# rohitsinghlab/SAME

Hardware: AMD Instinct MI355X
Metric: cell-pairs/sec on 100k×100k cost build + edge-cross sweep; % HBM roofline (higher is better)
Workload: dtype f64

## Files before the change

include/same_hip.h:

```cpp
#ifndef SAME_HIP_H
#define SAME_HIP_H

#include <stddef.h>
#include <stdint.h>

#ifdef __cplusplus
extern "C" {
#endif

#define SAME_OK 0
#define SAME_EINVAL (-22)
#define SAME_ENOMEM (-12)
#define SAME_EIO (-5)
#define SAME_ENODEV (-19)
#define SAME_ERANGE (-34)
#define SAME_EUNSURE (-11)

#define SAME_ABI_VERSION 8
#define SAME_MAX_KNN 448
#define SAME_MAX_TYPES 4096

typedef struct same_ctx same_ctx;
typedef struct same_sweep same_sweep;

// ... 128 lines not shown
                       int64_t Tr, const int32_t *dmatch, double *dout_before, double *dout_after,
                       uint8_t *dout_matched3, uint8_t *dout_flipped);
int same_xyorder_sweep_dev(same_ctx *ctx, const double *daxy, int64_t n_m, const double *drxy,
                           const int32_t *dtris, int64_t Tr, const int32_t *dmatch,
                           uint8_t *dedge_flags, uint8_t *dtri_flag, uint8_t *dpoint_flag,
                           uint64_t *dcounts);
int same_orient_sweep_dev(same_sweep *sweep, const int32_t *dmatch, int64_t *out_checked,
                          int32_t *out_viol_idx, int64_t *out_nviol);
int same_orient_flags_dev(same_sweep *sweep, const int32_t *dmatch, int64_t t_begin, int64_t t_end,
                          uint8_t *dflag);
int same_orient_from_flags_dev(same_sweep *sweep, const uint8_t *dflag, int64_t *out_checked,
                               int32_t *out_viol_idx, int64_t *out_nviol);
int same_first_candidate_dev(same_ctx *ctx, const int32_t *didx, int64_t rows, int k, int32_t *dmatch);

#define SAME_WINDOW_BATCH_MAX 64
typedef struct same_section same_section;
typedef struct same_window same_window;
enum {
    SAME_WINDOW_ALIGNED_XY = 0,
    SAME_WINDOW_ALIGNED_ROWS = 1,
    SAME_WINDOW_ROWS_M = 2,
    SAME_WINDOW_ROWS_R = 3,
    SAME_WINDOW_PAIRS = 4,
    SAME_WINDOW_COSTS = 5,
    SAME_WINDOW_KEPT = 6,
    SAME_WINDOW_SIGNS = 7,
    SAME_WINDOW_WEIGHTS = 8,
    SAME_WINDOW_MATCH = 9,
    SAME_WINDOW_TRIANGLES = 10
};
// ... 94 lines not shown
```

include/same_hip_diag.h:

```cpp
#ifndef SAME_HIP_DIAG_H
#define SAME_HIP_DIAG_H

#include "same_hip.h"

#ifdef __cplusplus
extern "C" {
#endif

enum { SAME_STAT_LAUNCHES = 0, SAME_STAT_FILLS = 1, SAME_STAT_COPIES = 2, SAME_STAT_WAITS = 3, SAME_STAT_GREEDY_READBACKS = 4, SAME_STAT_COUNT = 5 };
int same_ctx_stat(same_ctx *ctx, int which, int64_t *out);


int same_timer_start(same_ctx *ctx);
int same_timer_stop(same_ctx *ctx, float *out_ms);
int same_timer_mark(same_ctx *ctx);
int same_timer_read(same_ctx *ctx, float *out_ms);

int same_ctx_pci_bus_id(same_ctx *ctx, char *out, size_t out_len);
int same_dev_mem_info(same_ctx *ctx, int64_t *out_free, int64_t *out_total);

#define SAME_SPREAD_INFO_LEN 14
int same_dev_alloc_spread(same_ctx *ctx, size_t bytes, void **out_dptr, int64_t *out_info);

#define SAME_Q32_MAX_TYPES 32
int same_quantize_u32_dev(same_ctx *ctx, const double *dsrc, int64_t n, double offset, double scale,
// ... 13 lines not shown
```

same_amd/_lib.py:

```python
import ctypes
import os
import sys
import threading

import numpy as np

_HERE = os.path.dirname(os.path.abspath(__file__))
LIB_PATH = os.environ.get("SAME_HIP_LIB") or os.path.join(_HERE, "libsame_hip.so")

c_i64 = ctypes.c_int64
c_int = ctypes.c_int
c_dbl = ctypes.c_double
c_flt = ctypes.c_float
c_vp = ctypes.c_void_p
c_sz = ctypes.c_size_t

UNIQUE_ID_BYTES = 128
ABI_VERSION = 8
DT_U8, DT_I32, DT_U64, DT_F64 = 0, 1, 2, 3
OP_SUM, OP_MAX, OP_MIN = 0, 1, 2
SPREAD_INFO_LEN = 14
MAX_KNN = 448
MAX_TYPES = 4096

_PROTOTYPES = {
    "same_abi_version": [],
    "same_device_count": [ctypes.POINTER(c_int)],
    "same_ctx_create": [c_int, ctypes.POINTER(c_vp)],
    "same_ctx_destroy": [c_vp],
    "same_ctx_sync": [c_vp],
    "same_strerror": [c_int],
    "same_last_error": [c_vp],
    "same_ctx_info": [c_vp, ctypes.c_char_p, c_sz, ctypes.POINTER(c_int), ctypes.POINTER(c_i64)],
    "same_ctx_pci_bus_id": [c_vp, ctypes.c_char_p, c_sz],
    "same_ctx_stat": [c_vp, c_int, ctypes.POINTER(c_i64)],
    "same_dev_alloc": [c_vp, c_sz, ctypes.POINTER(c_vp)],
    "same_dev_free": [c_vp, c_vp],
    "same_dev_alloc_spread": [c_vp, c_sz, ctypes.POINTER(c_vp), ctypes.POINTER(c_i64)],
    "same_h2d": [c_vp, c_vp, c_vp, c_sz],
    "same_d2h": [c_vp, c_vp, c_vp, c_sz],
    "same_dev_memset": [c_vp, c_vp, c_int, c_sz],
    "same_d2d": [c_vp, c_vp, c_vp, c_sz],
    "same_dev_mem_info": [c_vp, ctypes.POINTER(c_i64), ctypes.POINTER(c_i64)],
    "same_ctx_release_scratch": [c_vp],
    "same_timer_start": [c_vp],
    "same_timer_stop": [c_vp, ctypes.POINTER(c_flt)],
    "same_timer_mark": [c_vp],
    "same_timer_read": [c_vp, ctypes.POINTER(c_flt)],
    "same_pair_cost_f64": [c_vp, c_vp, c_vp, c_i64, c_i64, c_int, c_vp, c_vp, c_vp, c_i64, c_dbl, c_vp],
    "same_pair_cost_f32": [c_vp, c_vp, c_vp, c_i64, c_i64, c_int, c_vp, c_vp, c_vp, c_i64, c_flt, c_vp],
# ... 73 lines not shown
    "same_comm_destroy": [c_vp],
    "same_allgather_dev": [c_vp, c_vp, c_vp, c_sz],
    "same_allgather_dev_async": [c_vp, c_vp, c_vp, c_sz],
    "same_comm_wait": [c_vp],
    "same_allreduce_dev": [c_vp, c_vp, c_sz, c_int, c_int],
    "same_comm_group_start": [c_vp],
    "same_comm_group_end": [c_vp],
    "same_comm_info": [c_vp, ctypes.POINTER(c_int), ctypes.POINTER(c_int), ctypes.POINTER(c_int)],
    "same_comm_device": [c_vp, ctypes.POINTER(c_int)],
    "same_comm_gather_time": [c_vp, ctypes.POINTER(c_flt), ctypes.POINTER(c_i64)],
}
EXPORTS = tuple(_PROTOTYPES)


SAME_EINVAL, SAME_ENOMEM, SAME_EIO, SAME_ENODEV, SAME_ERANGE, SAME_EUNSURE = -22, -12, -5, -19, -34, -11
SAME_DD_FEW_POINTS, SAME_DD_NO_ANGLE, SAME_DD_NONFINITE, SAME_DD_IN_DOUBT, SAME_DD_OVERFLOW = 1, 2, 4, 8, 16


class SameHipError(RuntimeError):

    def __init__(self, code, what, detail=""):
        self.code = code
        super().__init__(f"{what}: {detail}" if detail else what)


_lib = None
_lib_lock = threading.Lock()


def load():
# ... 213 lines not shown
```

same_amd/csrc/common.h:

```cpp
#pragma once
#include <hip/hip_runtime.h>

#include <cstdint>
#include <cstdio>
#include <cstring>
#include <string>
#include <vector>

#include "same_hip_diag.h"

struct ncclComm;

enum Slot {
    SL_A = 0, SL_R, SL_AXY, SL_RXY, SL_PAIRS, SL_OUT0, SL_OUT1, SL_OUT2, SL_TRIS, SL_MATCH,
    SL_SIGN, SL_SIZE, SL_TYPE, SL_FLAG0, SL_FLAG1, SL_FLAG2, SL_COUNTS, SL_X, SL_MASK,
    SL_K_HIST, SL_K_RANK, SL_K_SXY, SL_K_SIDX, SL_K_BBOX, SL_K_START,
    SL_COUNT
};

struct same_spread_alloc {
    char *va = nullptr;
    size_t bytes = 0;
    std::vector<void *> handles;
};
void same_spread_release(same_spread_alloc &a);

struct same_ctx {
    int device = -1;
    hipStream_t stream = nullptr;
    hipStream_t comm_stream = nullptr;
    hipEvent_t ev0 = nullptr, ev1 = nullptr;
    hipEvent_t ev_ready = nullptr, ev_gathered = nullptr;
    hipEvent_t ev_gather0 = nullptr;
    bool gather_open = false, gather_stamped = false, in_group = false;
    size_t gather_bytes = 0;
    void *slot[SL_COUNT] = {};
    size_t slot_bytes[SL_COUNT] = {};
    void *pinned = nullptr;
    size_t pinned_bytes = 0;
    std::string err;
    int cu_count = 0;
    ncclComm *comm = nullptr;
    int nranks = 1, rank = 0;
    std::vector<same_spread_alloc> spread;
    int64_t stats[SAME_STAT_COUNT] = {};
};

#define SAME_LAUNCH(ctx, kernel, grid, block, lds, ...)                                  \
    do {                                                                                 \
        ++(ctx)->stats[SAME_STAT_LAUNCHES];                                              \
        hipLaunchKernelGGL(kernel, grid, block, lds, (ctx)->stream, __VA_ARGS__);        \
    } while (0)
#define SAME_FILL(ctx, ptr, value, bytes)                                                \
    do {                                                                                 \
// ... 67 lines not shown
    void *p = nullptr;
    int rc = same_slot(ctx, s, n * sizeof(T), &p);
    *out = static_cast<T *>(p);
    return rc;
}
template <typename T>
inline int up_as(same_ctx *ctx, Slot s, const T *host, size_t n, T **out) {
    void *p = nullptr;
    int rc = same_up(ctx, s, host, n * sizeof(T), &p);
    *out = static_cast<T *>(p);
    return rc;
}

static inline int64_t ceil_div(int64_t a, int64_t b) { return (a + b - 1) / b; }

int check_index_range(same_ctx *ctx, const int32_t *idx, int64_t n, int64_t lo, int64_t hi, const char *what);

int same_pair_rowmin_core(same_ctx *ctx, const int32_t *dpairs, const double *dcosts, int64_t P, int64_t n_m, double *dout);
int same_greedy_core(same_ctx *ctx, const int32_t *dpairs, const double *dcosts, int64_t P, int64_t n_m, int64_t n_r,
                     const uint8_t *dprefer, int32_t *dmatch_pair, int *out_rounds);

constexpr int SAME_GREEDY_BATCH_MAX = 64;
struct same_greedy_state {
    uint8_t *alive = nullptr;
    uint8_t *used = nullptr;
    unsigned long long *key[2] = {nullptr, nullptr};
    unsigned *idx[2] = {nullptr, nullptr};
    unsigned long long *sel = nullptr;
    bool float_costs = false;
};
// ... 38 lines not shown
```

same_amd/csrc/ctx.hip:

```cpp
#include "common.h"

extern "C" {

int same_abi_version(void) { return SAME_ABI_VERSION; }

int same_device_count(int *out_count) {
    if (!out_count) return SAME_EINVAL;
    int n = 0;
    hipError_t e = hipGetDeviceCount(&n);
    if (e != hipSuccess) { *out_count = 0; return SAME_ENODEV; }
    *out_count = n;
    return SAME_OK;
}

int same_ctx_create(int device, same_ctx **out) {
    if (!out) return SAME_EINVAL;
    *out = nullptr;
    int n = 0;
    if (hipGetDeviceCount(&n) != hipSuccess || n <= 0) return SAME_ENODEV;
    if (device < 0 || device >= n) return SAME_EINVAL;
    same_ctx *ctx = new (std::nothrow) same_ctx();
    if (!ctx) return SAME_ENOMEM;
    ctx->device = device;
    hipError_t e = hipSetDevice(device);
// ... 13 lines not shown
    ctx->cu_count = prop.multiProcessorCount;
    *out = ctx;
    return SAME_OK;
}

void same_ctx_destroy(same_ctx *ctx) {
    if (!ctx) return;
    (void)hipSetDevice(ctx->device);
    if (ctx->comm) same_comm_destroy(ctx);
    if (ctx->stream) (void)hipStreamSynchronize(ctx->stream);
    if (ctx->comm_stream) (void)hipStreamSynchronize(ctx->comm_stream);
    for (int s = 0; s < SL_COUNT; ++s)
        if (ctx->slot[s]) (void)hipFree(ctx->slot[s]);
    for (auto &a : ctx->spread) same_spread_release(a);
    if (ctx->pinned) (void)hipHostFree(ctx->pinned);
    if (ctx->ev0) (void)hipEventDestroy(ctx->ev0);
    if (ctx->ev1) (void)hipEventDestroy(ctx->ev1);
    if (ctx->ev_ready) (void)hipEventDestroy(ctx->ev_ready);
    if (ctx->ev_gathered) (void)hipEventDestroy(ctx->ev_gathered);
    if (ctx->ev_gather0) (void)hipEventDestroy(ctx->ev_gather0);
    if (ctx->comm_stream) (void)hipStreamDestroy(ctx->comm_stream);
    if (ctx->stream) (void)hipStreamDestroy(ctx->stream);
    delete ctx;
}

int same_ctx_sync(same_ctx *ctx) {
    REQUIRE(ctx, ctx != nullptr);
    SAME_TRY(same_use(ctx));
    HIP_TRY(ctx, hipStreamSynchronize(ctx->stream));
    HIP_TRY(ctx, hipStreamSynchronize(ctx->comm_stream));
// ... 25 lines not shown
    return SAME_OK;
}

int same_ctx_pci_bus_id(same_ctx *ctx, char *out, size_t out_len) {
    REQUIRE(ctx, ctx && out && out_len >= 16 && out_len <= 4096);
    HIP_TRY(ctx, hipDeviceGetPCIBusId(out, (int)out_len, ctx->device));
    return SAME_OK;
}

int same_ctx_stat(same_ctx *ctx, int which, int64_t *out) {
    REQUIRE(ctx, ctx && out && which >= 0 && which < SAME_STAT_COUNT);
    *out = ctx->stats[which];
    return SAME_OK;
}

int same_dev_alloc(same_ctx *ctx, size_t bytes, void **out_dptr) {
    REQUIRE(ctx, ctx && out_dptr);
    SAME_TRY(same_use(ctx));
    *out_dptr = nullptr;
    HIP_TRY(ctx, hipMalloc(out_dptr, bytes ? bytes : 1));
    return SAME_OK;
}

int same_dev_free(same_ctx *ctx, void *dptr) {
    REQUIRE(ctx, ctx != nullptr);
    SAME_TRY(same_use(ctx));
    HIP_TRY(ctx, hipStreamSynchronize(ctx->stream));
    for (size_t i = 0; i < ctx->spread.size(); ++i)
        if (ctx->spread[i].va == dptr) {
            same_spread_release(ctx->spread[i]);
// ... 136 lines not shown
```

same_amd/csrc/window_finish.hip:

```cpp
#include "assign.h"
#include "refine.h"

namespace {

using namespace devmath;
using namespace win;
using scan::Pair;

struct FilterArgs {
    const double *xy;
    const int32_t *raw;
    int64_t Tr, n;
    const int32_t *type_id;
    uint8_t *cls;
    double *perim;
    uint8_t *has_kept, *any_valid;
    unsigned long long *best_p;
    unsigned *best_t, *first_v;
    unsigned long long *st_keep, *st_own, *counters;
    int32_t *klist, *nlist, *out;
};

__global__ __launch_bounds__(256) void filter_classify_kernel(Batch<FilterArgs> b, double radius, int angle_enabled, double cos_thr, int near_enabled,
                                                               double tol) {
    const FilterArgs &w = b.w[blockIdx.y];
    if ((int64_t)blockIdx.x * blockDim.x >= w.Tr) return;
    const int64_t t = (int64_t)blockIdx.x * blockDim.x + threadIdx.x;
    const int32_t *__restrict__ tris = w.raw, *__restrict__ type_id = w.type_id;
    bool near = false;
    if (t < w.Tr) {
        const int32_t a = tris[3 * t], bb = tris[3 * t + 1], d = tris[3 * t + 2];
        const TriClass r = classify_triangle(ld2(w.xy, a), ld2(w.xy, bb), ld2(w.xy, d), radius, angle_enabled, cos_thr,
                                             type_id && type_id[a] == type_id[bb] && type_id[bb] == type_id[d]);
        w.cls[t] = r.cls;
        w.perim[t] = r.perim;
        near = near_enabled && r.cls != 1 && fabs(r.maxcos - cos_thr) <= tol;
        if (r.cls == 0 || r.cls == 3) {
            w.any_valid[a] = 1; w.any_valid[bb] = 1; w.any_valid[d] = 1;
            if (r.cls == 0) { w.has_kept[a] = 1; w.has_kept[bb] = 1; w.has_kept[d] = 1; }
        }
        if (w.best_p && r.cls == 3) {
            const unsigned long long key = ~(unsigned long long)__double_as_longlong(r.perim);
            atomicMax(&w.best_p[a], key); atomicMax(&w.best_p[bb], key); atomicMax(&w.best_p[d], key);
        }
    }
    const unsigned long long nb = __ballot(near);
    if ((threadIdx.x & 63) == 0 && nb) atomicAdd(&w.counters[FC_NEAR], (unsigned long long)__builtin_popcountll(nb));
}
__global__ __launch_bounds__(scan::NT) void filter_keep_kernel(Batch<FilterArgs> b) {
    __shared__ scan::Shared sh;
    const FilterArgs &w = b.w[blockIdx.y];
    const int nb = (int)scan::blocks_for(w.Tr);
    if ((int)blockIdx.x >= nb || w.Tr == 0) return;
    const int64_t Tr = w.Tr;
    const uint8_t *__restrict__ cls = w.cls;
    auto val = [&](int64_t t) { return Pair{t < Tr && cls[t] == 0 ? 1u : 0u, 0u}; };
    Pair through;
    const Pair off = scan::exclusive(w.st_keep, (int)blockIdx.x, val, sh, &through);
    const int64_t t = (int64_t)blockIdx.x * scan::NT + threadIdx.x;
    if (t < Tr) {
        const uint8_t c = cls[t];
        if (c == 0) w.klist[off.a] = (int32_t)t;
// ... 182 lines not shown
    __syncthreads();
    if (threadIdx.x < 7) {
        const int s = part[0][threadIdx.x] + part[1][threadIdx.x] + part[2][threadIdx.x] + part[3][threadIdx.x];
        if (s) atomicAdd(&counters[threadIdx.x < 6 ? threadIdx.x : SC_TIES], (unsigned long long)s);
    }
}

struct FilterPlan {
    FilterArgs args{};
    void *zero = nullptr;
    size_t zero_bytes = 0;
    unsigned long long *counters = nullptr;
    bool readd = false;
};

int prepare_filter(same_window *w, const int32_t *d_simplices, int64_t Tr, int ignore_same_type, int ensure_min_triangle_per_node, FilterPlan *plan) {
    same_ctx *ctx = w->ctx;
    const int64_t n = w->n_ua;
    const bool use_type = ignore_same_type && w->has_type;
    plan->readd = use_type && ensure_min_triangle_per_node;
    Carver cv;
    const size_t st_keep = scan::status_bytes(Tr), st_own = scan::status_bytes(n);
    const size_t o_st_keep = cv.take(st_keep), o_st_own = cv.take(st_own), o_counters = cv.take(64), o_has_kept = cv.take((size_t)n),
                 o_any_valid = cv.take((size_t)n), o_best_p = cv.take((size_t)n * 8), o_best_t = cv.take((size_t)n * 4),
                 o_first_v = cv.take((size_t)Tr * 4);
    const size_t zero_bytes = cv.off;
    const size_t o_cls = cv.take((size_t)Tr), o_perim = cv.take((size_t)Tr * 8), o_klist = cv.take((size_t)Tr * 4), o_nlist = cv.take((size_t)n * 4);
    SAME_TRY(ensure(ctx, w->filter, cv.off));
    SAME_TRY(ensure(ctx, w->tris, (size_t)std::max<int64_t>(Tr, 1) * 12));
    char *base = static_cast<char *>(w->filter.p);
    auto at = [&](size_t off) { return base + off; };
    unsigned long long *dc = reinterpret_cast<unsigned long long *>(at(o_counters));
    plan->counters = dc;
    FilterArgs &a = plan->args;
    a.xy = w->axy_c;
    a.raw = d_simplices;
    a.Tr = Tr;
    a.n = n;
    a.type_id = use_type ? w->type_c : nullptr;
    a.cls = reinterpret_cast<uint8_t *>(at(o_cls));
    a.perim = reinterpret_cast<double *>(at(o_perim));
    a.has_kept = reinterpret_cast<uint8_t *>(at(o_has_kept));
    a.any_valid = reinterpret_cast<uint8_t *>(at(o_any_valid));
    a.best_p = plan->readd ? reinterpret_cast<unsigned long long *>(at(o_best_p)) : nullptr;
    a.best_t = reinterpret_cast<unsigned *>(at(o_best_t));
    a.first_v = reinterpret_cast<unsigned *>(at(o_first_v));
    a.st_keep = scan::arg(reinterpret_cast<unsigned long long *>(at(o_st_keep)));
    a.st_own = scan::arg(reinterpret_cast<unsigned long long *>(at(o_st_own)));
    a.counters = dc;
    a.klist = reinterpret_cast<int32_t *>(at(o_klist));
// ... 275 lines not shown
                if (q < batch) break;
                if (batch < SAME_GREEDY_BATCH_MAX) batch *= 2;
            }
            again = true;
        }
    }
    SAME_TRY(settle(w, p, again));
    for (int q = 0; q < 8; ++q) out_stats[q] = (int64_t)cnt[q];
    out_stats[SC_ROUNDS] = rounds;
    *out_ties += (int64_t)cnt[SC_TIES];
    memcpy(out_match_row, h + p->o_match_row, (size_t)n * sizeof(int32_t));
    memcpy(out_point_flag, h + p->o_pflag, (size_t)n);
    return SAME_OK;
}

int filter_finish(same_window *const *windows, int n_windows, const int32_t *simplices, const int64_t *simplex_offsets, int prefiltered,
                  bool on_device, double radius, int angle_enabled, double cos_thr, double near_tol, int ignore_same_type,
                  int ensure_min_triangle_per_node, double no_match_penalty, int32_t *out_match_row, uint8_t *out_point_flag,
                  int64_t *out_stats, int64_t *out_counts) {
    same_ctx *ctx = nullptr;
    SAME_TRY(check_batch(windows, n_windows, &ctx));
    REQUIRE(ctx, simplex_offsets && out_counts && out_stats && simplex_offsets[0] == 0);
    int64_t n_cells = 0;
    for (int i = 0; i < n_windows; ++i) {
        const int64_t Tr = simplex_offsets[i + 1] - simplex_offsets[i];
        REQUIRE(ctx, windows[i]->staged == 2 && Tr >= 0 && Tr < ((int64_t)1 << 31) - 512);
        n_cells += windows[i]->n_ua;
    }
    REQUIRE(ctx, (simplex_offsets[n_windows] == 0 || simplices || on_device) && (n_cells == 0 || (out_match_row && out_point_flag)));
    for (int q = 0; q < 4 * n_windows; ++q) out_counts[q] = 0;
    for (int q = 0; q < 8 * n_windows; ++q) out_stats[q] = 0;
    SAME_TRY(same_use(ctx));
    if (!on_device)
        for (int i = 0; i < n_windows; ++i)
            SAME_TRY(check_index_range(ctx, simplices + 3 * simplex_offsets[i], (simplex_offsets[i + 1] - simplex_offsets[i]) * 3, 0,
                                       windows[i]->n_ua, "triangles"));
    struct Item {
        FilterPlan fplan;
        FinishPlan plan;
        bool filtered = false, enqueued = false;
    };
    std::vector<Item> items((size_t)n_windows);
    const int32_t *d_simplices = nullptr;
    if (!on_device && !prefiltered && simplex_offsets[n_windows] > 0) {
        int32_t *d = nullptr;
        SAME_TRY(slot_as(ctx, SL_TRIS, (size_t)simplex_offsets[n_windows] * 3, &d));
        SAME_COPY(ctx, d, simplices, (size_t)simplex_offsets[n_windows] * 12, hipMemcpyHostToDevice);
        d_simplices = d;
    }
    int rc = SAME_OK;
    std::vector<same_window *> live;
    std::vector<FinishPlan *> plans;
    std::vector<FilterPlan *> fplans;
    for (int i = 0; i < n_windows && rc == SAME_OK; ++i) {
        same_window *w = windows[i];
        Item &it = items[(size_t)i];
        const int32_t *tri = on_device ? nullptr : simplices + 3 * simplex_offsets[i];
        const int64_t Tr = simplex_offsets[i + 1] - simplex_offsets[i];
        w->filtered = w->finished = 0;
        w->Tr = 0;
        w->as_rounds = w->as_flags = 0;
        w->as_objective = 0.0;
        w->rf_rounds = w->rf_moves = w->rf_settled = 0;
        w->rf_obj0 = w->rf_obj = 0.0;
        w->rf_nm = no_match_penalty;
        if (w->n_ua == 0) continue;
        if (Tr && !prefiltered) {
            const int32_t *raw = on_device ? static_cast<const int32_t *>(w->dd_tris.p) : d_simplices + 3 * simplex_offsets[i];
            rc = prepare_filter(w, raw, Tr, ignore_same_type, ensure_min_triangle_per_node, &it.fplan);
            if (rc == SAME_OK) rc = prepare_finish(w, nullptr, Tr, it.fplan.counters + FC_TR, &it.plan);
            if (rc == SAME_OK) {
                fplans.push_back(&it.fplan);
                it.plan.filter_zero = it.fplan.zero;
                it.plan.filter_zero_bytes = it.fplan.zero_bytes;
            }
            it.filtered = true;
        } else {
            rc = prepare_finish(w, Tr ? tri : nullptr, Tr, nullptr, &it.plan);
        }
        if (rc == SAME_OK) {
            live.push_back(w);
            plans.push_back(&it.plan);
        }
    }
    for (size_t g = 0; g < live.size() && rc == SAME_OK; g += SAME_LAUNCH_WINDOWS) {
        ZeroArgs zr[SAME_LAUNCH_WINDOWS];
        const int n_g = (int)std::min<size_t>(SAME_LAUNCH_WINDOWS, live.size() - g);
        for (int q = 0; q < n_g; ++q) {
            const FinishPlan *fp = plans[g + (size_t)q];
            zr[q] = ZeroArgs{{fp->zero, fp->filter_zero}, {fp->zero_bytes, fp->filter_zero_bytes}};
        }
        rc = launch_zero(ctx, zr, n_g);
    }
    for (size_t g = 0, e; g < fplans.size() && rc == SAME_OK; g = e) {
        for (e = g + 1; e < fplans.size() && e - g < SAME_LAUNCH_WINDOWS && fplans[e]->readd == fplans[g]->readd; ++e) {}
        rc = launch_filter(ctx, fplans.data() + g, (int)(e - g), radius, angle_enabled, cos_thr, near_tol);
    }
    for (size_t g = 0, e; g < live.size() && rc == SAME_OK; g = e) {
        for (e = g + 1; e < live.size() && e - g < SAME_LAUNCH_WINDOWS && live[e]->cost_f32 == live[g]->cost_f32 &&
// ... 20 lines not shown
                    }
                    if (rc == SAME_OK) rc = enqueue_finish_copy(w, &it.plan);
                }
                it.enqueued = rc == SAME_OK;
            }
            if (rc == SAME_OK && n_g && (n_g == SAME_LAUNCH_WINDOWS || i == n_windows - 1)) {
                rc = launch_copy_back(ctx, ca, n_g);
                n_g = 0;
            }
        }
    }
    if (rc != SAME_OK) {
        (void)hipStreamSynchronize(ctx->stream);
        return rc;
    }
    SAME_WAIT(ctx);
    int64_t cell0 = 0;
    for (int i = 0; i < n_windows; ++i) {
        same_window *w = windows[i];
        Item &it = items[(size_t)i];
        const int64_t Tr = simplex_offsets[i + 1] - simplex_offsets[i];
        int64_t *counts = out_counts + 4 * i, *stats = out_stats + 8 * i;
        if (!it.enqueued) {
            w->filtered = w->finished = 1;
            continue;
        }
        int32_t *const match_out = out_match_row + cell0;
        uint8_t *const flag_out = out_point_flag + cell0;
        cell0 += w->n_ua;
        if (it.filtered) {
            const unsigned long long *hf = reinterpret_cast<const unsigned long long *>(static_cast<const char *>(w->host) + w->host_filter_off);
// ... 2 lines not shown
            counts[1] = n_add;
            counts[2] = n_near;
            counts[3] = (int64_t)hf[FC_TIES];
            if (n_near) {
                for (int q = 0; q < 8; ++q) stats[q] = 0;
                continue;
            }
            w->Tr = n_keep + n_add;
        } else {
            counts[0] = Tr;
            w->Tr = Tr;
        }
        SAME_TRY(read_finish(w, &it.plan, match_out, flag_out, stats, counts + 3));
        w->filtered = w->finished = 1;
    }
    return SAME_OK;
}

}

extern "C" {

int same_window_filter_finish(same_window *const *windows, int n_windows, const int32_t *simplices, const int64_t *simplex_offsets, int prefiltered,
                              double radius, int angle_enabled, double cos_thr, double near_tol, int ignore_same_type,
                              int ensure_min_triangle_per_node, double no_match_penalty, int32_t *out_match_row, uint8_t *out_point_flag,
                              int64_t *out_stats, int64_t *out_counts) {
    return filter_finish(windows, n_windows, simplices, simplex_offsets, prefiltered, false, radius, angle_enabled, cos_thr, near_tol,
                         ignore_same_type, ensure_min_triangle_per_node, no_match_penalty, out_match_row, out_point_flag, out_stats, out_counts);
}

int same_window_filter_finish_device(same_window *const *windows, int n_windows, double radius, int angle_enabled, double cos_thr, double near_tol,
                                     int ignore_same_type, int ensure_min_triangle_per_node, double no_match_penalty, int32_t *out_match_row,
                                     uint8_t *out_point_flag, int64_t *out_stats, int64_t *out_counts) {
    same_ctx *ctx = nullptr;
    SAME_TRY(check_batch(windows, n_windows, &ctx));
    std::vector<int64_t> offsets((size_t)n_windows + 1, 0);
    for (int i = 0; i < n_windows; ++i) {
        REQUIRE(ctx, windows[i]->dd_ok && windows[i]->staged == 2);
        offsets[(size_t)i + 1] = offsets[(size_t)i] + windows[i]->n_dd;
    }
    return filter_finish(windows, n_windows, nullptr, offsets.data(), 0, true, radius, angle_enabled, cos_thr, near_tol, ignore_same_type,
                         ensure_min_triangle_per_node, no_match_penalty, out_match_row, out_point_flag, out_stats, out_counts);
}
// ... 66 lines not shown
```

same_amd/csrc/window_internal.h:

```cpp
#pragma once
#include <algorithm>
#include <cmath>
#include <memory>
#include <mutex>
#include <new>
#include <shared_mutex>
#include <utility>
#include <vector>

#include "common.h"
#include "devmath.h"
#include "scan.h"

struct same_knn_index;
extern "C" int same_knn_index_build(same_ctx *ctx, const double *drxy, int64_t n_r, double radius, same_knn_index **out);
extern "C" void same_knn_index_destroy(same_knn_index *ix);

namespace win {

constexpr int MAX_RUN_CELLS = 64;
constexpr int64_t MAX_GRID_CELLS = (int64_t)1 << 22;
constexpr unsigned OUTSIDE = 0x80000000u;

struct DevBuf {
// ... 41 lines not shown
struct Batch {
    A w[SAME_LAUNCH_WINDOWS];
};

struct ZeroArgs {
    void *p[2];
    size_t bytes[2];
};

struct CopyArgs {
    const void *src[2];
    void *dst[2];
    size_t bytes[2];
};

struct Cover {
    int cx0 = 0, ncx = 0, cy0 = 0, ncy = 0;
    int64_t n_cand = 0;
    bool aligned = false, use_runs = false;
};

enum { FC_KEEP = 0, FC_ADD = 1, FC_NEAR = 2, FC_TR = 3, FC_TIES = 4, FC_COPIED = 5 };
enum { SC_CHECKED = 0, SC_FLIPPED = 1, SC_CMP = 2, SC_VIOL = 3, SC_TVIOL = 4, SC_AFLIP = 5, SC_ROUNDS = 6, SC_MATCHED = 7, SC_REMAINING = 8, SC_TIES = 9,
       SC_REFINE = 16, SC_COUNT = 32 };

}

struct same_section {
    same_ctx *ctx = nullptr;
    int64_t n = 0;
    int T = 0;
    int cost_f32 = 0;
    double *xy = nullptr;
    void *xy_c = nullptr;
    void *types_c = nullptr;
    double *types64 = nullptr;
    double *size = nullptr;
// ... 57 lines not shown
```

same_amd/csrc/window_stage.hip:

```cpp
#include "window_internal.h"

namespace {

using namespace devmath;
using namespace win;
using scan::Pair;

__global__ __launch_bounds__(256) void zero_kernel(Batch<ZeroArgs> b) {
    const ZeroArgs &w = b.w[blockIdx.y];
    typedef unsigned u4 __attribute__((ext_vector_type(4)));
#pragma unroll
    for (int r = 0; r < 2; ++r) {
        const size_t n16 = w.bytes[r] >> 4;
        u4 *dst = static_cast<u4 *>(w.p[r]);
        for (size_t i = (size_t)blockIdx.x * blockDim.x + threadIdx.x; i < n16; i += (size_t)gridDim.x * blockDim.x) dst[i] = u4{0u, 0u, 0u, 0u};
        if (blockIdx.x == 0 && threadIdx.x < (w.bytes[r] & 15)) static_cast<char *>(w.p[r])[(n16 << 4) + threadIdx.x] = 0;
    }
}

__global__ __launch_bounds__(256) void copy_back_kernel(Batch<CopyArgs> b) {
    const CopyArgs &w = b.w[blockIdx.y];
    typedef unsigned u4 __attribute__((ext_vector_type(4)));
#pragma unroll
    for (int r = 0; r < 2; ++r) {
// ... 535 lines not shown
    REQUIRE(ctx, w->n_m <= w->cap_m && w->n_r <= w->cap_r && w->n_ua <= w->n_m && w->P <= (int64_t)sp.slots);
    out_counts[0] = w->n_m;
    out_counts[1] = w->n_r;
    out_counts[2] = w->n_ua;
    out_counts[3] = w->P;
    w->staged = (w->n_m && w->n_r) ? 2 : 1;
    return SAME_OK;
}

}

extern "C" {

int same_window_stage(same_window *const *windows, int n_windows, const same_section *mov, const same_section *ref, const double *boxes,
                      double radius, int k, double dist_ct_coeff, int64_t *out_counts) {
    same_ctx *ctx = nullptr;
    SAME_TRY(check_batch(windows, n_windows, &ctx));
    REQUIRE(ctx, mov && ref && boxes && out_counts && mov->ctx->device == ctx->device && ref->ctx->device == ctx->device);
    REQUIRE(ctx, mov->T == ref->T && mov->cost_f32 == ref->cost_f32 && k >= 1 && k <= SAME_MAX_KNN && radius >= 0.0);
    SAME_TRY(same_use(ctx));
    for (int i = 0; i < 4 * n_windows; ++i) out_counts[i] = 0;
    for (int i = 0; i < n_windows; ++i) windows[i]->staged = windows[i]->finished = windows[i]->filtered = windows[i]->dd_ok = 0;
    std::shared_ptr<same_knn_index> ix;
    SAME_TRY(knn_index_for(ctx, ref, radius, &ix));
    std::shared_lock<std::shared_mutex> grid_m(const_cast<same_section *>(mov)->grid_lock), grid_r;
    if (ref != mov) grid_r = std::shared_lock<std::shared_mutex>(const_cast<same_section *>(ref)->grid_lock);
    std::vector<StagePlan> plans((size_t)n_windows);
    int rc = SAME_OK;
    for (int i = 0; i < n_windows && rc == SAME_OK; ++i) rc = prepare_stage(windows[i], mov, ref, boxes + 4 * i, k, &plans[(size_t)i]);
    for (int g = 0; g < n_windows && rc == SAME_OK; g += SAME_LAUNCH_WINDOWS) {
// ... 11 lines not shown
            if (w->host_dev) {
                ca[q] = CopyArgs{{w->counts, nullptr}, {w->host_dev, nullptr}, {plans[(size_t)(g + q)].back_bytes, 0}};
                continue;
            }
            hipError_t e = hipMemcpyAsync(w->host, w->counts, plans[(size_t)(g + q)].back_bytes, hipMemcpyDeviceToHost, ctx->stream);
            ++ctx->stats[SAME_STAT_COPIES];
            if (e != hipSuccess) rc = same_fail(ctx, SAME_EIO, "stage copy back", e);
        }
        if (rc == SAME_OK) rc = launch_copy_back(ctx, ca, n_g);
    }
    if (rc != SAME_OK) {
        (void)hipStreamSynchronize(ctx->stream);
        for (int i = 0; i < n_windows; ++i) windows[i]->staged = 0;
        return rc;
    }
    SAME_WAIT(ctx);
    for (int i = 0; i < n_windows; ++i) SAME_TRY(collect_stage(windows[i], plans[(size_t)i], out_counts + 4 * i));
    return SAME_OK;
}

int same_window_fetch(same_window *w, int what, void *out, int64_t bytes) {
    if (!w) return SAME_EINVAL;
    same_ctx *ctx = w->ctx;
    REQUIRE(ctx, w->staged >= 1 && bytes >= 0 && (bytes == 0 || out));
    SAME_TRY(same_use(ctx));
    const char *h = static_cast<const char *>(w->host);
    const void *dev = nullptr;
    const void *host = nullptr;
    int64_t want = 0;
    const int64_t n_m = w->n_m, n_r = w->n_r, n_ua = w->n_ua, P = w->P, Tr = w->Tr;
    const bool full = w->staged == 2;
// ... 27 lines not shown
```

same_amd/delaunay.py:

```python
import os
import threading
from concurrent.futures import ThreadPoolExecutor

import numpy as np

from . import _lib, qhull_pool

GUARD = 16.0


def mode(optim_params=None):
    m = (optim_params or {}).get("hip_delaunay") or os.environ.get("SAME_DELAUNAY") or "qhull"
    m = str(m).lower()
    if m not in ("native", "device", "qhull"):
        raise ValueError(f"hip_delaunay / SAME_DELAUNAY must be 'native', 'device' or 'qhull', not {m!r}")
    return m


def device_filtered_triangles(points, radius, min_angle_deg, ctx=None, guard=GUARD, with_status=False):
    import ctypes

    from . import ops
    from .triangles import cos_threshold

    ctx = ops._ctx(ctx)
    pts = np.ascontiguousarray(points, dtype=np.float64).reshape(-1, 2)
    n = len(pts)
    angle_enabled, cos_thr = cos_threshold(min_angle_deg)
    out = np.empty((max(2 * n, 1), 3), np.int32)
    n_tris, status = ctypes.c_int64(0), ctypes.c_int(0)
    with ctx.lock:
        ctx.check(ctx.lib.same_delaunay_filtered(ctx.handle, pts.ctypes.data, n, float(abs(radius)), int(angle_enabled), float(cos_thr),
                                                 float(guard), out.ctypes.data, len(out), ctypes.byref(n_tris), ctypes.byref(status)),
                  "same_delaunay_filtered")
    tris = None if status.value else out[:n_tris.value].copy()
    return (tris, status.value) if with_status else tris


def native_simplices(points, guard=GUARD, with_margin=False):
    import ctypes

    lib = _lib.load()
    pts = np.ascontiguousarray(points, dtype=np.float64).reshape(-1, 2)
    n = len(pts)
    out = np.empty((max(2 * n - 5, 1), 3), np.int32)
    n_tris, margin = ctypes.c_int64(0), ctypes.c_double(0.0)
    rc = lib.same_delaunay2d(pts.ctypes.data, n, out.ctypes.data, len(out), ctypes.byref(n_tris), float(guard), ctypes.byref(margin))
    if rc == _lib.SAME_EUNSURE:
        return (None, margin.value) if with_margin else None
    if rc != 0:
        raise _lib.SameHipError(rc, "same_delaunay2d")
    tris = out[:n_tris.value]
    return (tris, margin.value) if with_margin else tris


class Ticket:

    def __init__(self, owner, points, pending=None, simplices=None, native=False, key=None):
        self.owner, self.points, self.key = owner, points, key
        self._pending, self._simplices, self.native = pending, simplices, native
# ... 172 lines not shown
```

same_amd/windows.py:

```python
import os

import numpy as np

from . import ops
from .delaunay import QHULL, QhullTriangulator, Ticket


def window_grid(ref_xy, mov_xy, window_size, overlap):
    import warnings

    with warnings.catch_warnings():
        warnings.simplefilter("ignore", RuntimeWarning)
        x_min = min(np.nanmin(ref_xy[:, 0]), np.nanmin(mov_xy[:, 0]))
        x_max = max(np.nanmax(ref_xy[:, 0]), np.nanmax(mov_xy[:, 0]))
        y_min = min(np.nanmin(ref_xy[:, 1]), np.nanmin(mov_xy[:, 1]))
        y_max = max(np.nanmax(ref_xy[:, 1]), np.nanmax(mov_xy[:, 1]))
    step = window_size - overlap
    xs = list(range(int(x_min), int(x_max), step))
    ys = list(range(int(y_min), int(y_max), step))
    return xs, ys, (x_min, x_max, y_min, y_max)


def _candidate_boxes(xs, ys, ws):
    boxes = np.empty((len(xs), len(ys), 4, 4), np.float64)
# ... 625 lines not shown

def stage_windows(states, moving, ref, boxes, radius, knn, dist_ct_coeff):
    ctx, n = states[0].ctx, len(states)
    boxes = np.ascontiguousarray(boxes, dtype=np.float64).reshape(n, 4)
    counts = np.zeros((n, 4), np.int64)
    with ctx.lock:
        ctx.check(ctx.lib.same_window_stage(_handles(states), n, moving.handle, ref.handle, boxes.ctypes.data, float(radius), int(knn),
                                            float(dist_ct_coeff), counts.ctypes.data), "same_window_stage")
    for s, c in zip(states, counts.tolist()):
        s.counts, s.n_triangles = tuple(c), 0
    return [s.counts for s in states]


def filter_finish_windows(states, simplices, radius, angle_enabled, cos_thr, near_tol, ignore_same_type, no_match_penalty,
                          ensure_min_triangle_per_node=True, prefiltered=False):
    ctx, n = states[0].ctx, len(states)
    tris = [ops._tris(t) for t in simplices]
    offsets = np.zeros(n + 1, np.int64)
    np.cumsum([len(t) for t in tris], out=offsets[1:])
    flat = tris[0] if n == 1 else np.concatenate(tris)

    def call(match_row, flag, stats, counts):
        return ctx.lib.same_window_filter_finish(_handles(states), n, flat.ctypes.data, offsets.ctypes.data, int(bool(prefiltered)),
                                                 float(radius),
                                                 int(angle_enabled), float(cos_thr), float(near_tol), int(bool(ignore_same_type)),
                                                 int(bool(ensure_min_triangle_per_node)), float(no_match_penalty), match_row.ctypes.data,
                                                 flag.ctypes.data, stats.ctypes.data, counts.ctypes.data)

    return _filter_finish_results(states, call, "same_window_filter_finish")


def filter_finish_device_windows(states, radius, angle_enabled, cos_thr, near_tol, ignore_same_type, no_match_penalty,
                                 ensure_min_triangle_per_node=True):
    ctx, n = states[0].ctx, len(states)

    def call(match_row, flag, stats, counts):
        return ctx.lib.same_window_filter_finish_device(_handles(states), n, float(radius), int(angle_enabled), float(cos_thr),
                                                        float(near_tol), int(bool(ignore_same_type)), int(bool(ensure_min_triangle_per_node)),
# ... 220 lines not shown
```

Before: 612.6 billion.

## Pass per-window simplex pointers and read pinned triangles directly on device

The filter-finish path now receives an array of per-window triangle pointers instead of one concatenated host buffer. Triangulation output goes into page-locked blocks, so the filter kernel can read triangles through their device-mapped addresses and copy them into the device slot itself. Non-pinned windows are staged through a reused pinned host buffer. The host-side index range check is replaced by an in-kernel bad-index flag that is checked after the wait. Phase timing counters are added, which costs a few clock reads per call, and mapped host reads from the kernel may be slower than a bulk copy.

```diff
diff --git a/include/same_hip.h b/include/same_hip.h
--- a/include/same_hip.h
+++ b/include/same_hip.h
@@ -166,6 +166,7 @@
 int same_first_candidate_dev(same_ctx *ctx, const int32_t *didx, int64_t rows, int k, int32_t *dmatch);
 
 #define SAME_WINDOW_BATCH_MAX 64
+#define SAME_SIMPLICES_PER_WINDOW 2
 typedef struct same_section same_section;
 typedef struct same_window same_window;
 enum {
diff --git a/include/same_hip_diag.h b/include/same_hip_diag.h
--- a/include/same_hip_diag.h
+++ b/include/same_hip_diag.h
@@ -9,6 +9,11 @@
 
 enum { SAME_STAT_LAUNCHES = 0, SAME_STAT_FILLS = 1, SAME_STAT_COPIES = 2, SAME_STAT_WAITS = 3, SAME_STAT_GREEDY_READBACKS = 4, SAME_STAT_COUNT = 5 };
 int same_ctx_stat(same_ctx *ctx, int which, int64_t *out);
+
+enum { SAME_PHASE_FF_CALLS = 0, SAME_PHASE_FF_TOTAL = 1, SAME_PHASE_FF_CHECK = 2, SAME_PHASE_FF_PLAN = 3, SAME_PHASE_FF_UPLOAD = 4,
+       SAME_PHASE_FF_ENQUEUE = 5, SAME_PHASE_FF_WAIT = 6, SAME_PHASE_FF_READ = 7, SAME_PHASE_ST_CALLS = 8, SAME_PHASE_ST_TOTAL = 9,
+       SAME_PHASE_ST_WAIT = 10, SAME_PHASE_FF_STAGED = 11, SAME_PHASE_COUNT = 12 };
+int same_window_phase_ns(int64_t *out, int n, int reset);
 
 
 int same_timer_start(same_ctx *ctx);
diff --git a/same_amd/_lib.py b/same_amd/_lib.py
--- a/same_amd/_lib.py
+++ b/same_amd/_lib.py
@@ -34,6 +34,7 @@
     "same_ctx_info": [c_vp, ctypes.c_char_p, c_sz, ctypes.POINTER(c_int), ctypes.POINTER(c_i64)],
     "same_ctx_pci_bus_id": [c_vp, ctypes.c_char_p, c_sz],
     "same_ctx_stat": [c_vp, c_int, ctypes.POINTER(c_i64)],
+    "same_window_phase_ns": [ctypes.POINTER(c_i64), c_int, c_int],
     "same_dev_alloc": [c_vp, c_sz, ctypes.POINTER(c_vp)],
     "same_dev_free": [c_vp, c_vp],
     "same_dev_alloc_spread": [c_vp, c_sz, ctypes.POINTER(c_vp), ctypes.POINTER(c_i64)],
@@ -137,6 +138,7 @@
 
 
 SAME_EINVAL, SAME_ENOMEM, SAME_EIO, SAME_ENODEV, SAME_ERANGE, SAME_EUNSURE = -22, -12, -5, -19, -34, -11
+SAME_SIMPLICES_PER_WINDOW = 2
 SAME_DD_FEW_POINTS, SAME_DD_NO_ANGLE, SAME_DD_NONFINITE, SAME_DD_IN_DOUBT, SAME_DD_OVERFLOW = 1, 2, 4, 8, 16
 
 
diff --git a/same_amd/csrc/common.h b/same_amd/csrc/common.h
--- a/same_amd/csrc/common.h
+++ b/same_amd/csrc/common.h
@@ -38,6 +38,8 @@
     size_t slot_bytes[SL_COUNT] = {};
     void *pinned = nullptr;
     size_t pinned_bytes = 0;
+    void *tri_host = nullptr;
+    size_t tri_host_bytes = 0;
     std::string err;
     int cu_count = 0;
     ncclComm *comm = nullptr;
@@ -135,6 +137,10 @@
 
 static inline int64_t ceil_div(int64_t a, int64_t b) { return (a + b - 1) / b; }
 
+int64_t same_phase_add(int which, int64_t t0);
+int64_t same_phase_now();
+void same_phase_bump(int which);
+
 int check_index_range(same_ctx *ctx, const int32_t *idx, int64_t n, int64_t lo, int64_t hi, const char *what);
 
 int same_pair_rowmin_core(same_ctx *ctx, const int32_t *dpairs, const double *dcosts, int64_t P, int64_t n_m, double *dout);
diff --git a/same_amd/csrc/ctx.hip b/same_amd/csrc/ctx.hip
--- a/same_amd/csrc/ctx.hip
+++ b/same_amd/csrc/ctx.hip
@@ -1,4 +1,21 @@
 #include "common.h"
+
+#include <atomic>
+#include <chrono>
+
+namespace {
+std::atomic<int64_t> g_phase_ns[SAME_PHASE_COUNT];
+}
+
+int64_t same_phase_now() {
+    return std::chrono::duration_cast<std::chrono::nanoseconds>(std::chrono::steady_clock::now().time_since_epoch()).count();
+}
+int64_t same_phase_add(int which, int64_t t0) {
+    const int64_t t = same_phase_now();
+    g_phase_ns[which].fetch_add(t - t0, std::memory_order_relaxed);
+    return t;
+}
+void same_phase_bump(int which) { g_phase_ns[which].fetch_add(1, std::memory_order_relaxed); }
 
 extern "C" {
 
@@ -51,6 +68,7 @@
         if (ctx->slot[s]) (void)hipFree(ctx->slot[s]);
     for (auto &a : ctx->spread) same_spread_release(a);
     if (ctx->pinned) (void)hipHostFree(ctx->pinned);
+    if (ctx->tri_host) (void)hipHostFree(ctx->tri_host);
     if (ctx->ev0) (void)hipEventDestroy(ctx->ev0);
     if (ctx->ev1) (void)hipEventDestroy(ctx->ev1);
     if (ctx->ev_ready) (void)hipEventDestroy(ctx->ev_ready);
@@ -106,6 +124,14 @@
     return SAME_OK;
 }
 
+int same_window_phase_ns(int64_t *out, int n, int reset) {
+    if (!out || n < 0 || n > SAME_PHASE_COUNT) return SAME_EINVAL;
+    for (int q = 0; q < n; ++q) out[q] = g_phase_ns[q].load(std::memory_order_relaxed);
+    if (reset)
+        for (int q = 0; q < SAME_PHASE_COUNT; ++q) g_phase_ns[q].store(0, std::memory_order_relaxed);
+    return SAME_OK;
+}
+
 int same_dev_alloc(same_ctx *ctx, size_t bytes, void **out_dptr) {
     REQUIRE(ctx, ctx && out_dptr);
     SAME_TRY(same_use(ctx));
diff --git a/same_amd/csrc/window_finish.hip b/same_amd/csrc/window_finish.hip
--- a/same_amd/csrc/window_finish.hip
+++ b/same_amd/csrc/window_finish.hip
@@ -9,7 +9,8 @@
 
 struct FilterArgs {
     const double *xy;
-    const int32_t *raw;
+    const int32_t *src;
+    int32_t *raw;
     int64_t Tr, n;
     const int32_t *type_id;
     uint8_t *cls;
@@ -26,10 +27,25 @@
     const FilterArgs &w = b.w[blockIdx.y];
     if ((int64_t)blockIdx.x * blockDim.x >= w.Tr) return;
     const int64_t t = (int64_t)blockIdx.x * blockDim.x + threadIdx.x;
-    const int32_t *__restrict__ tris = w.raw, *__restrict__ type_id = w.type_id;
-    bool near = false;
+    const int32_t *tris = w.src, *__restrict__ type_id = w.type_id;
+    bool near = false, bad = false;
+    int32_t a = 0, bb = 0, d = 0;
     if (t < w.Tr) {
-        const int32_t a = tris[3 * t], bb = tris[3 * t + 1], d = tris[3 * t + 2];
+        a = tris[3 * t];
+        bb = tris[3 * t + 1];
+        d = tris[3 * t + 2];
+        if (tris != w.raw) {
+            w.raw[3 * t] = a;
+            w.raw[3 * t + 1] = bb;
+            w.raw[3 * t + 2] = d;
+        }
+        bad = a < 0 || a >= w.n || bb < 0 || bb >= w.n || d < 0 || d >= w.n;
+        if (bad) {
+            w.cls[t] = 1;
+            w.perim[t] = 0.0;
+        }
+    }
+    if (!bad && t < w.Tr) {
         const TriClass r = classify_triangle(ld2(w.xy, a), ld2(w.xy, bb), ld2(w.xy, d), radius, angle_enabled, cos_thr,
                                              type_id && type_id[a] == type_id[bb] && type_id[bb] == type_id[d]);
         w.cls[t] = r.cls;
@@ -44,8 +60,9 @@
             atomicMax(&w.best_p[a], key); atomicMax(&w.best_p[bb], key); atomicMax(&w.best_p[d], key);
         }
     }
-    const unsigned long long nb = __ballot(near);
+    const unsigned long long nb = __ballot(near), any_bad = __ballot(bad);
     if ((threadIdx.x & 63) == 0 && nb) atomicAdd(&w.counters[FC_NEAR], (unsigned long long)__builtin_popcountll(nb));
+    if ((threadIdx.x & 63) == 0 && any_bad) atomicOr(&w.counters[FC_BAD], 1ull);
 }
 __global__ __launch_bounds__(scan::NT) void filter_keep_kernel(Batch<FilterArgs> b) {
     __shared__ scan::Shared sh;
@@ -258,7 +275,7 @@
     bool readd = false;
 };
 
-int prepare_filter(same_window *w, const int32_t *d_simplices, int64_t Tr, int ignore_same_type, int ensure_min_triangle_per_node, FilterPlan *plan) {
+int prepare_filter(same_window *w, int32_t *d_simplices, const int32_t *src, int64_t Tr, int ignore_same_type, int ensure_min_triangle_per_node, FilterPlan *plan) {
     same_ctx *ctx = w->ctx;
     const int64_t n = w->n_ua;
     const bool use_type = ignore_same_type && w->has_type;
@@ -278,6 +295,7 @@
     plan->counters = dc;
     FilterArgs &a = plan->args;
     a.xy = w->axy_c;
+    a.src = src;
     a.raw = d_simplices;
     a.Tr = Tr;
     a.n = n;
@@ -583,10 +601,48 @@
     return SAME_OK;
 }
 
-int filter_finish(same_window *const *windows, int n_windows, const int32_t *simplices, const int64_t *simplex_offsets, int prefiltered,
+int place_simplices(same_ctx *ctx, const int32_t *const *tri, const int64_t *offsets, int n_windows, int32_t *d,
+                    std::vector<const int32_t *> &src, std::vector<int32_t *> &raw) {
+    int64_t lo = -1, hi = 0;
+    for (int i = 0; i < n_windows; ++i) {
+        raw[(size_t)i] = d + 3 * offsets[i];
+        src[(size_t)i] = nullptr;
+        if (offsets[i + 1] == offsets[i]) continue;
+        void *dev = nullptr;
+        if (hipHostGetDevicePointer(&dev, const_cast<int32_t *>(tri[i]), 0) == hipSuccess && dev) {
+            src[(size_t)i] = static_cast<const int32_t *>(dev);
+            continue;
+        }
+        (void)hipGetLastError();
+        if (lo < 0) lo = offsets[i];
+        hi = offsets[i + 1];
+    }
+    if (lo < 0) return SAME_OK;
+    same_phase_bump(SAME_PHASE_FF_STAGED);
+    const size_t bytes = (size_t)offsets[n_windows] * 12;
+    if (ctx->tri_host_bytes < bytes) {
+        if (ctx->tri_host) HIP_TRY(ctx, hipHostFree(ctx->tri_host));
+        ctx->tri_host = nullptr;
+        ctx->tri_host_bytes = 0;
+        const size_t want = std::max<size_t>(bytes + bytes / 4, (size_t)1 << 20);
+        HIP_TRY(ctx, hipHostMalloc(&ctx->tri_host, want, hipHostMallocDefault));
+        ctx->tri_host_bytes = want;
+    }
+    int32_t *h = static_cast<int32_t *>(ctx->tri_host);
+    for (int i = 0; i < n_windows; ++i)
+        if (offsets[i + 1] > offsets[i] && !src[(size_t)i]) {
+            memcpy(h + 3 * offsets[i], tri[i], (size_t)(offsets[i + 1] - offsets[i]) * 12);
+            src[(size_t)i] = raw[(size_t)i];
+        }
+    SAME_COPY(ctx, d + 3 * lo, h + 3 * lo, (size_t)(hi - lo) * 12, hipMemcpyHostToDevice);
+    return SAME_OK;
+}
+
+int filter_finish(same_window *const *windows, int n_windows, const int32_t *const *tri, const int64_t *simplex_offsets, int prefiltered,
                   bool on_device, double radius, int angle_enabled, double cos_thr, double near_tol, int ignore_same_type,
                   int ensure_min_triangle_per_node, double no_match_penalty, int32_t *out_match_row, uint8_t *out_point_flag,
                   int64_t *out_stats, int64_t *out_counts) {
+    PhaseClock clock(SAME_PHASE_FF_CALLS, SAME_PHASE_FF_TOTAL);
     same_ctx *ctx = nullptr;
     SAME_TRY(check_batch(windows, n_windows, &ctx));
     REQUIRE(ctx, simplex_offsets && out_counts && out_stats && simplex_offsets[0] == 0);
@@ -596,27 +652,31 @@
         REQUIRE(ctx, windows[i]->staged == 2 && Tr >= 0 && Tr < ((int64_t)1 << 31) - 512);
         n_cells += windows[i]->n_ua;
     }
-    REQUIRE(ctx, (simplex_offsets[n_windows] == 0 || simplices || on_device) && (n_cells == 0 || (out_match_row && out_point_flag)));
+    REQUIRE(ctx, (simplex_offsets[n_windows] == 0 || tri || on_device) && (n_cells == 0 || (out_match_row && out_point_flag)));
+    if (!on_device)
+        for (int i = 0; i < n_windows; ++i) REQUIRE(ctx, simplex_offsets[i + 1] == simplex_offsets[i] || tri[i]);
     for (int q = 0; q < 4 * n_windows; ++q) out_counts[q] = 0;
     for (int q = 0; q < 8 * n_windows; ++q) out_stats[q] = 0;
     SAME_TRY(same_use(ctx));
     if (!on_device)
         for (int i = 0; i < n_windows; ++i)
-            SAME_TRY(check_index_range(ctx, simplices + 3 * simplex_offsets[i], (simplex_offsets[i + 1] - simplex_offsets[i]) * 3, 0,
-                                       windows[i]->n_ua, "triangles"));
+            if (prefiltered || windows[i]->n_ua == 0)
+                SAME_TRY(check_index_range(ctx, tri[i], (simplex_offsets[i + 1] - simplex_offsets[i]) * 3, 0, windows[i]->n_ua, "triangles"));
+    clock.lap(SAME_PHASE_FF_CHECK);
     struct Item {
         FilterPlan fplan;
         FinishPlan plan;
         bool filtered = false, enqueued = false;
     };
     std::vector<Item> items((size_t)n_windows);
-    const int32_t *d_simplices = nullptr;
+    std::vector<const int32_t *> src((size_t)n_windows, nullptr);
+    std::vector<int32_t *> raw((size_t)n_windows, nullptr);
     if (!on_device && !prefiltered && simplex_offsets[n_windows] > 0) {
         int32_t *d = nullptr;
         SAME_TRY(slot_as(ctx, SL_TRIS, (size_t)simplex_offsets[n_windows] * 3, &d));
-        SAME_COPY(ctx, d, simplices, (size_t)simplex_offsets[n_windows] * 12, hipMemcpyHostToDevice);
-        d_simplices = d;
-    }
+        SAME_TRY(place_simplices(ctx, tri, simplex_offsets, n_windows, d, src, raw));
+    }
+    clock.lap(SAME_PHASE_FF_UPLOAD);
     int rc = SAME_OK;
     std::vector<same_window *> live;
     std::vector<FinishPlan *> plans;
@@ -624,7 +684,6 @@
     for (int i = 0; i < n_windows && rc == SAME_OK; ++i) {
         same_window *w = windows[i];
         Item &it = items[(size_t)i];
-        const int32_t *tri = on_device ? nullptr : simplices + 3 * simplex_offsets[i];
         const int64_t Tr = simplex_offsets[i + 1] - simplex_offsets[i];
         w->filtered = w->finished = 0;
         w->Tr = 0;
@@ -635,8 +694,8 @@
         w->rf_nm = no_match_penalty;
         if (w->n_ua == 0) continue;
         if (Tr && !prefiltered) {
-            const int32_t *raw = on_device ? static_cast<const int32_t *>(w->dd_tris.p) : d_simplices + 3 * simplex_offsets[i];
-            rc = prepare_filter(w, raw, Tr, ignore_same_type, ensure_min_triangle_per_node, &it.fplan);
+            int32_t *d = on_device ? static_cast<int32_t *>(w->dd_tris.p) : raw[(size_t)i];
+            rc = prepare_filter(w, d, on_device ? d : src[(size_t)i], Tr, ignore_same_type, ensure_min_triangle_per_node, &it.fplan);
             if (rc == SAME_OK) rc = prepare_finish(w, nullptr, Tr, it.fplan.counters + FC_TR, &it.plan);
             if (rc == SAME_OK) {
                 fplans.push_back(&it.fplan);
@@ -645,13 +704,14 @@
             }
             it.filtered = true;
         } else {
-            rc = prepare_finish(w, Tr ? tri : nullptr, Tr, nullptr, &it.plan);
+            rc = prepare_finish(w, Tr ? tri[i] : nullptr, Tr, nullptr, &it.plan);
         }
         if (rc == SAME_OK) {
             live.push_back(w);
             plans.push_back(&it.plan);
         }
     }
+    clock.lap(SAME_PHASE_FF_PLAN);
     for (size_t g = 0; g < live.size() && rc == SAME_OK; g += SAME_LAUNCH_WINDOWS) {
         ZeroArgs zr[SAME_LAUNCH_WINDOWS];
         const int n_g = (int)std::min<size_t>(SAME_LAUNCH_WINDOWS, live.size() - g);
@@ -702,7 +762,18 @@
         (void)hipStreamSynchronize(ctx->stream);
         return rc;
     }
+    clock.lap(SAME_PHASE_FF_ENQUEUE);
     SAME_WAIT(ctx);
+    clock.lap(SAME_PHASE_FF_WAIT);
+    for (int i = 0; i < n_windows; ++i) {
+        const same_window *w = windows[i];
+        if (!items[(size_t)i].filtered || !reinterpret_cast<const unsigned long long *>(static_cast<const char *>(w->host) + w->host_filter_off)[FC_BAD])
+            continue;
+        if (!on_device)
+            SAME_TRY(check_index_range(ctx, tri[i], (simplex_offsets[i + 1] - simplex_offsets[i]) * 3, 0, w->n_ua, "triangles"));
+        ctx->err = "triangles: an index outside the window's kept cells";
+        return SAME_ERANGE;
+    }
     int64_t cell0 = 0;
     for (int i = 0; i < n_windows; ++i) {
         same_window *w = windows[i];
@@ -735,6 +806,7 @@
         SAME_TRY(read_finish(w, &it.plan, match_out, flag_out, stats, counts + 3));
         w->filtered = w->finished = 1;
     }
+    clock.lap(SAME_PHASE_FF_READ);
     return SAME_OK;
 }
 
@@ -746,8 +818,17 @@
                               double radius, int angle_enabled, double cos_thr, double near_tol, int ignore_same_type,
                               int ensure_min_triangle_per_node, double no_match_penalty, int32_t *out_match_row, uint8_t *out_point_flag,
                               int64_t *out_stats, int64_t *out_counts) {
-    return filter_finish(windows, n_windows, simplices, simplex_offsets, prefiltered, false, radius, angle_enabled, cos_thr, near_tol,
-                         ignore_same_type, ensure_min_triangle_per_node, no_match_penalty, out_match_row, out_point_flag, out_stats, out_counts);
+    same_ctx *ctx = nullptr;
+    SAME_TRY(check_batch(windows, n_windows, &ctx));
+    REQUIRE(ctx, simplex_offsets);
+    const int32_t *tri[SAME_WINDOW_BATCH_MAX];
+    const bool each = (prefiltered & SAME_SIMPLICES_PER_WINDOW) != 0;
+    for (int i = 0; i < n_windows; ++i)
+        tri[i] = !simplices ? nullptr : each ? reinterpret_cast<const int32_t *const *>(simplices)[i] : simplices + 3 * simplex_offsets[i];
+    prefiltered = (prefiltered & ~SAME_SIMPLICES_PER_WINDOW) != 0;
+    return filter_finish(windows, n_windows, simplices ? tri : nullptr, simplex_offsets, prefiltered, false, radius, angle_enabled, cos_thr,
+                         near_tol, ignore_same_type, ensure_min_triangle_per_node, no_match_penalty, out_match_row, out_point_flag, out_stats,
+                         out_counts);
 }
 
 int same_window_filter_finish_device(same_window *const *windows, int n_windows, double radius, int angle_enabled, double cos_thr, double near_tol,
diff --git a/same_amd/csrc/window_internal.h b/same_amd/csrc/window_internal.h
--- a/same_amd/csrc/window_internal.h
+++ b/same_amd/csrc/window_internal.h
@@ -79,13 +79,21 @@
     size_t bytes[2];
 };
 
+struct PhaseClock {
+    int64_t t0, t;
+    int total;
+    PhaseClock(int calls, int total_) : t0(same_phase_now()), t(t0), total(total_) { same_phase_bump(calls); }
+    ~PhaseClock() { same_phase_add(total, t0); }
+    void lap(int which) { t = same_phase_add(which, t); }
+};
+
 struct Cover {
     int cx0 = 0, ncx = 0, cy0 = 0, ncy = 0;
     int64_t n_cand = 0;
     bool aligned = false, use_runs = false;
 };
 
-enum { FC_KEEP = 0, FC_ADD = 1, FC_NEAR = 2, FC_TR = 3, FC_TIES = 4, FC_COPIED = 5 };
+enum { FC_KEEP = 0, FC_ADD = 1, FC_NEAR = 2, FC_TR = 3, FC_TIES = 4, FC_BAD = 5, FC_COPIED = 6 };
 enum { SC_CHECKED = 0, SC_FLIPPED = 1, SC_CMP = 2, SC_VIOL = 3, SC_TVIOL = 4, SC_AFLIP = 5, SC_ROUNDS = 6, SC_MATCHED = 7, SC_REMAINING = 8, SC_TIES = 9,
        SC_REFINE = 16, SC_COUNT = 32 };
 
diff --git a/same_amd/csrc/window_stage.hip b/same_amd/csrc/window_stage.hip
--- a/same_amd/csrc/window_stage.hip
+++ b/same_amd/csrc/window_stage.hip
@@ -573,6 +573,7 @@
 
 int same_window_stage(same_window *const *windows, int n_windows, const same_section *mov, const same_section *ref, const double *boxes,
                       double radius, int k, double dist_ct_coeff, int64_t *out_counts) {
+    PhaseClock clock(SAME_PHASE_ST_CALLS, SAME_PHASE_ST_TOTAL);
     same_ctx *ctx = nullptr;
     SAME_TRY(check_batch(windows, n_windows, &ctx));
     REQUIRE(ctx, mov && ref && boxes && out_counts && mov->ctx->device == ctx->device && ref->ctx->device == ctx->device);
@@ -614,7 +615,9 @@
         for (int i = 0; i < n_windows; ++i) windows[i]->staged = 0;
         return rc;
     }
+    clock.t = same_phase_now();
     SAME_WAIT(ctx);
+    clock.lap(SAME_PHASE_ST_WAIT);
     for (int i = 0; i < n_windows; ++i) SAME_TRY(collect_stage(windows[i], plans[(size_t)i], out_counts + 4 * i));
     return SAME_OK;
 }
diff --git a/same_amd/delaunay.py b/same_amd/delaunay.py
--- a/same_amd/delaunay.py
+++ b/same_amd/delaunay.py
@@ -37,13 +37,40 @@
     return (tris, status.value) if with_status else tris
 
 
+_simplex_blocks, _simplex_blocks_lock = None, threading.Lock()
+
+
+def _page_locked_rows(rows):
+    global _simplex_blocks
+    if _simplex_blocks is False:
+        return None
+    if _simplex_blocks is None:
+        from .windows import _PinnedBlocks
+
+        class _SimplexBlocks(_PinnedBlocks):
+            KEEP, LIMIT = 128, 128
+
+        with _simplex_blocks_lock:
+            if _simplex_blocks is None:
+                _simplex_blocks = _SimplexBlocks() if _lib.device_count() > 0 else False
+        if _simplex_blocks is False:
+            return None
+    got = _simplex_blocks.take(_lib.default_context(), rows * 12)
+    if got is None:
+        return None
+    return np.frombuffer(got[0], np.int32, count=rows * 3).reshape(rows, 3)
+
+
 def native_simplices(points, guard=GUARD, with_margin=False):
     import ctypes
 
     lib = _lib.load()
     pts = np.ascontiguousarray(points, dtype=np.float64).reshape(-1, 2)
     n = len(pts)
-    out = np.empty((max(2 * n - 5, 1), 3), np.int32)
+    rows = max(2 * n - 5, 1)
+    out = _page_locked_rows(rows)
+    if out is None:
+        out = np.empty((rows, 3), np.int32)
     n_tris, margin = ctypes.c_int64(0), ctypes.c_double(0.0)
     rc = lib.same_delaunay2d(pts.ctypes.data, n, out.ctypes.data, len(out), ctypes.byref(n_tris), float(guard), ctypes.byref(margin))
     if rc == _lib.SAME_EUNSURE:
diff --git a/same_amd/windows.py b/same_amd/windows.py
--- a/same_amd/windows.py
+++ b/same_amd/windows.py
@@ -2,7 +2,7 @@
 
 import numpy as np
 
-from . import ops
+from . import _lib, ops
 from .delaunay import QHULL, QhullTriangulator, Ticket
 
 
@@ -663,14 +663,17 @@
 
 def filter_finish_windows(states, simplices, radius, angle_enabled, cos_thr, near_tol, ignore_same_type, no_match_penalty,
                           ensure_min_triangle_per_node=True, prefiltered=False):
+    import ctypes
+
     ctx, n = states[0].ctx, len(states)
     tris = [ops._tris(t) for t in simplices]
     offsets = np.zeros(n + 1, np.int64)
     np.cumsum([len(t) for t in tris], out=offsets[1:])
-    flat = tris[0] if n == 1 else np.concatenate(tris)
+    ptrs = (ctypes.c_void_p * n)(*[t.ctypes.data if len(t) else None for t in tris])
+    flags = int(bool(prefiltered)) | _lib.SAME_SIMPLICES_PER_WINDOW
 
     def call(match_row, flag, stats, counts):
-        return ctx.lib.same_window_filter_finish(_handles(states), n, flat.ctypes.data, offsets.ctypes.data, int(bool(prefiltered)),
+        return ctx.lib.same_window_filter_finish(_handles(states), n, ctypes.addressof(ptrs), offsets.ctypes.data, flags,
                                                  float(radius),
                                                  int(angle_enabled), float(cos_thr), float(near_tol), int(bool(ignore_same_type)),
                                                  int(bool(ensure_min_triangle_per_node)), float(no_match_penalty), match_row.ctypes.data,
```

Result: no change. 611.7 billion (median of 6 runs) (-0.1%).
